# zhuye98/ICL

Hardware: AMD Instinct MI355X
Metric: 3D volumes/sec/node (fwd+bwd, 96^3 patch) (higher is better)
Workload: dtype f32; 1 GPU; 3D U-Net ICL BraTS-shape synthetic 96x96x96, num_classes=2, batch=2 per GPU (1 labeled + 1 unlabeled), full ICL step incl. SGD; global_batch=2, parallelism=dp1, launch=hipGraph replay

## Files before the change

### icl_amd/csrc/icl_abi.inc

```

#include "kernels/common.h"
#include "kernels/norm.h"
#include "kernels/pool_resize.h"
#include "kernels/reduce.h"
#include "kernels/conv_mfma.h"
#include "kernels/conv_mfma_static.h"
#include "kernels/conv_mfma_flat.h"
#include "kernels/conv_bf16x3.h"
#include "kernels/conv_bf16x3_ws.h"
#include "kernels/conv_wgrad_tr.h"
#include "kernels/conv_wgrad_zs.h"
#include "kernels/conv_cin1.h"
#include "kernels/misc.h"
#include "kernels/loss.h"
#include "kernels/optim.h"
#include "kernels/adamw.h"
#include "kernels/winattn.h"
#include "kernels/linear_wgrad.h"
#include "kernels/token.h"
#include "kernels/gemm.h"
#include "kernels/datafeed.h"
#include "kernels/rankindex.h"
#include "kernels/prefix.h"
#include "kernels/intensity.h"
// ... 1760 lines not shown
  ICL_LAUNCH((icl::layernorm_bwd_wgrad_kernel<CPL, RU>), grid, dim3(256), 0, st, gy, x, gamma, mean, rstd, gx, part_g, part_b, (long)rows, c, rpb)
    if (c <= 64) ICL_LN_BW(1, 4);
    else if (c <= 128) ICL_LN_BW(2, 4);
    else if (c <= 256) ICL_LN_BW(4, 2);
    else if (c <= 512) ICL_LN_BW(8, 1);
    else ICL_LN_BW(16, 1);
#undef ICL_LN_BW
    int rc = check_launch("layernorm_bwd_wgrad");
    if (rc || !dgamma) return rc;
    const void* g[2] = {part_g, part_b};
    void* out[2] = {dgamma, dbeta};
    const int32_t rr[2] = {chunks, chunks}, cc[2] = {c, c};
    return icl_colsum_multi(g, out, rr, cc, 2, stream);
  }
  constexpr int longrow = 1;
  if (c >= 1024 && c <= 256 * 64 && longrow) {
    if (c <= 256 * 16) ICL_LAUNCH((icl::layernorm_bwd_longrow_kernel<16>), dim3((unsigned)rows), dim3(256), 0, st, gy, x, gamma, mean, rstd, gx, c);
    else if (c <= 256 * 32) ICL_LAUNCH((icl::layernorm_bwd_longrow_kernel<32>), dim3((unsigned)rows), dim3(256), 0, st, gy, x, gamma, mean, rstd, gx, c);
    else ICL_LAUNCH((icl::layernorm_bwd_longrow_kernel<64>), dim3((unsigned)rows), dim3(256), 0, st, gy, x, gamma, mean, rstd, gx, c);
  } else if (c >= 1024) {
    ICL_LAUNCH((icl::layernorm_bwd_kernel<true>), dim3((unsigned)rows), dim3(256), 0, st, gy, x, gamma, mean, rstd, gx, (long)rows, c);
  } else {
    ICL_LAUNCH((icl::layernorm_bwd_kernel<false>), dim3((unsigned)cdivl(rows, 4)), dim3(256), 0, st, gy, x, gamma, mean, rstd, gx,
               (long)rows, c);
  }
  int rc = check_launch("layernorm_bwd");
  if (rc || !ws) return rc;
  int cols = 256;
  while (cols > c && cols > 16) cols >>= 1;
  if (cols < c && cols < 256) cols <<= 1;
  ICL_LAUNCH(icl::layernorm_wgrad_kernel, dim3((c + cols - 1) / cols, (unsigned)chunks), dim3(256), 0, st, gy, x, mean, rstd, part_g, part_b,
             (long)rows, c, rpb, cols);
  rc = check_launch("layernorm_wgrad");
  if (rc || !dgamma) return rc;
  const void* g[2] = {part_g, part_b};
  void* out[2] = {dgamma, dbeta};
  const int32_t rr[2] = {chunks, chunks}, cc[2] = {c, c};
  return icl_colsum_multi(g, out, rr, cc, 2, stream);
}

int icl_gelu_fwd(const float* x, float* y, int64_t n, void* stream) {
  if (!x || !y || n < 1) return fail(-1, "gelu_fwd: bad argument");
  ICL_LAUNCH(icl::gelu_fwd_kernel, dim3(grid_for(n, 256)), dim3(256), 0, (hipStream_t)stream, x, y, (long)n);
  return check_launch("gelu_fwd");
}

int icl_gelu_bwd(const float* gy, const float* x, float* gx, int64_t n, void* stream) {
  if (!gy || !x || !gx || n < 1) return fail(-1, "gelu_bwd: bad argument");
  ICL_LAUNCH(icl::gelu_bwd_kernel, dim3(grid_for(n, 256)), dim3(256), 0, (hipStream_t)stream, gy, x, gx, (long)n);
  return check_launch("gelu_bwd");
}

static bool attn_class_tiles(int nc) {
  const char* e = getenv("ICL_ATTN_TILED");
  return nc > icl::kAttnMaxNc || (e && atoi(e) == 1);
}

int icl_attn_fwd(const float* q, const float* kv, float* logits, float* out, float* stats, int b, int h, int nc, int n, int d,
                 float scale, void* stream) {
  if (nc < 1 || nc > icl::kAttnMaxClasses) return fail(-1, "attn_fwd: %d classes (1 .. %d)", nc, icl::kAttnMaxClasses);
  if (!q || !kv || !logits || !out || !stats || b < 1 || h < 1 || n < 1 || (d != 8 && d != 16))
    return fail(-1, "attn_fwd: bad argument (head dim 8 or 16)");
  hipStream_t st = (hipStream_t)stream;
  const dim3 g1((n + 255) / 256, b * h), g2(b * h * nc);
  const bool tiled = attn_class_tiles(nc);
  if (d == 16) {
    if (tiled) ICL_LAUNCH((icl::attn_logits_kernel<16, true>), g1, dim3(256), 0, st, q, kv, logits, b, h, nc, n, scale);
    else ICL_LAUNCH((icl::attn_logits_kernel<16, false>), g1, dim3(256), 0, st, q, kv, logits, b, h, nc, n, scale);
    ICL_LAUNCH((icl::attn_softmax_pv_kernel<16, 256>), g2, dim3(256), 0, st, (const float*)logits, kv, out, stats, b, h, nc, n);
  } else {
    if (tiled) ICL_LAUNCH((icl::attn_logits_kernel<8, true>), g1, dim3(256), 0, st, q, kv, logits, b, h, nc, n, scale);
    else ICL_LAUNCH((icl::attn_logits_kernel<8, false>), g1, dim3(256), 0, st, q, kv, logits, b, h, nc, n, scale);
    ICL_LAUNCH((icl::attn_softmax_pv_kernel<8, 256>), g2, dim3(256), 0, st, (const float*)logits, kv, out, stats, b, h, nc, n);
  }
  return check_launch("attn_fwd");
}

int64_t icl_attn_bwd_ws_bytes(int b, int h, int nc, int n, int d) {
  if (b < 1 || h < 1 || nc < 1 || n < 1 || d < 1) return 0;
  return (int64_t)((n + 255) / 256) * b * h * nc * d * 4;
}

int icl_attn_bwd(const float* q, const float* kv, const float* logits, const float* stats, const float* out, const float* gout,
                 const float* glog, float* gq, float* gkv, int b, int h, int nc, int n, int d, float scale, void* stream) {
  return icl_attn_bwd_ws(q, kv, logits, stats, out, gout, glog, gq, gkv, nullptr, b, h, nc, n, d, scale, stream);
}

int icl_attn_bwd_ws(const float* q, const float* kv, const float* logits, const float* stats, const float* out, const float* gout,
                    const float* glog, float* gq, float* gkv, void* ws, int b, int h, int nc, int n, int d, float scale, void* stream) {
  if (nc < 1 || nc > icl::kAttnMaxClasses) return fail(-1, "attn_bwd: %d classes (1 .. %d)", nc, icl::kAttnMaxClasses);
  if (!q || !kv || !logits || !stats || !out || !gq || !gkv || b < 1 || h < 1 || n < 1 || (d != 8 && d != 16))
    return fail(-1, "attn_bwd: bad argument");
  hipStream_t st = (hipStream_t)stream;
  const dim3 g1((n + 255) / 256, b * h), g2(b * h * nc);
  float* pq = (float*)ws;
  const bool tiled = attn_class_tiles(nc);
  if (d == 16) {
    if (tiled) ICL_LAUNCH((icl::attn_bwd_kv_kernel<16, true>), g1, dim3(256), 0, st, q, kv, logits, stats, out, gout, glog, gkv, b, h, nc, n, scale, pq);
    else ICL_LAUNCH((icl::attn_bwd_kv_kernel<16, false>), g1, dim3(256), 0, st, q, kv, logits, stats, out, gout, glog, gkv, b, h, nc, n, scale, pq);
    if (!pq) ICL_LAUNCH((icl::attn_bwd_q_kernel<16, 256>), g2, dim3(256), 0, st, kv, logits, stats, out, gout, glog, gq, b, h, nc, n, scale);
  } else {
    if (tiled) ICL_LAUNCH((icl::attn_bwd_kv_kernel<8, true>), g1, dim3(256), 0, st, q, kv, logits, stats, out, gout, glog, gkv, b, h, nc, n, scale, pq);
    else ICL_LAUNCH((icl::attn_bwd_kv_kernel<8, false>), g1, dim3(256), 0, st, q, kv, logits, stats, out, gout, glog, gkv, b, h, nc, n, scale, pq);
    if (!pq) ICL_LAUNCH((icl::attn_bwd_q_kernel<8, 256>), g2, dim3(256), 0, st, kv, logits, stats, out, gout, glog, gq, b, h, nc, n, scale);
  }
  if (pq) {
    const int rd = b * h * nc * d;
    ICL_LAUNCH(icl::attn_dq_reduce_kernel, dim3((rd + 255) / 256), dim3(256), 0, st, (const float*)pq, gq, (int)g1.x, rd, scale);
  }
  return check_launch("attn_bwd");
}

int64_t icl_window_attn_bias_elems(int n, int heads) { return icl_window_attn_bias_elems_impl(n, heads); }

static int linear_wgrad_nsplit(int64_t rows, int o, int i) {
  const int ob = (o + icl::kLwB - 1) / icl::kLwB, ib = (i + icl::kLwB - 1) / icl::kLwB;
  long n = rows * (o + i) / ((long)o * i + o);
  const long want = (2048 + ob * ib - 1) / (ob * ib);
  if (n > want) n = want;
  const long steps = (rows + 3) / 4;
  if (n > steps / 8) n = steps / 8;
  if (n < 4) n = 4;
  return (int)((n + 3) / 4 * 4);
}

int64_t icl_linear_wgrad_ws_bytes(int64_t rows, int o, int i) {
  return (int64_t)linear_wgrad_nsplit(rows, o, i) * ((int64_t)o * i + o) * 4;
}

int icl_linear_wgrad(const float* gy, const float* x, float* dw, float* db, void* ws, int64_t rows, int o, int i, void* stream) {
  if (!gy || !x || !dw || !ws || rows < 1 || o < 1 || i < 1) return fail(-1, "linear_wgrad: bad argument");
  hipStream_t st = (hipStream_t)stream;
  const int nsplit = linear_wgrad_nsplit(rows, o, i);
  const int ob = (o + icl::kLwB - 1) / icl::kLwB, ib = (i + icl::kLwB - 1) / icl::kLwB;
  ICL_LAUNCH(icl::linear_wgrad_kernel, dim3(nsplit / 4, ob, ib), dim3(256), 0, st, gy, x, (float*)ws, (long)rows, o, i, nsplit);
  if (int rc = check_launch("linear_wgrad")) return rc;
  const long EW = (long)o * i, E = EW + o;
  ICL_LAUNCH(icl::linear_wgrad_reduce_kernel, dim3((unsigned)cdivl(E, 16)), dim3(256), 0, st, (const float*)ws, dw, db, E, EW, nsplit);
  return check_launch("linear_wgrad_reduce");
}

static bool cin1_geom(icl::Cin1Geom& g, int n, int cout, int d, int h, int w, int64_t xbs, int64_t ybs) {
  if (n < 1 || cout < 1 || cout > 16 || d < 1 || h < 1 || w < 1 || (long)d * h * w * 16 >= (1L << 31)) return false;
  g.N = n; g.Cout = cout; g.D = d; g.H = h; g.W = w; g.nty = (h + icl::kC1Rows - 1) / icl::kC1Rows;
  g.x_bstride = xbs; g.y_bstride = ybs; g.ntiles = n * d * g.nty;
  return (size_t)3 * (icl::kC1Rows + 2) * (w + 2) * 4 <= 64 * 1024;
}
static int cin1_grid(const icl::Cin1Geom& g) { return g.ntiles < 2048 ? g.ntiles : 2048; }
static size_t cin1_lds(const icl::Cin1Geom& g) {
  const size_t halo = (size_t)3 * (icl::kC1Rows + 2) * (g.W + 2) * 4;
  return halo > 2048 * 4 ? halo : 2048 * 4;
}

int icl_conv3d_cin1_fwd(const float* x, const float* w, const float* bias, float* y, int n, int cout, int d, int h, int wd, int64_t x_bstride,
                        int64_t y_bstride, void* stream) {
  icl::Cin1Geom g;
  if (!x || !w || !y || !cin1_geom(g, n, cout, d, h, wd, x_bstride, y_bstride)) return fail(-1, "conv3d_cin1_fwd: bad argument");
  ICL_LAUNCH(icl::conv_cin1_fwd_kernel, dim3(cin1_grid(g)), dim3(icl::kC1Threads), cin1_lds(g), (hipStream_t)stream, x, w, bias, y, g);
  snprintf(g_kernel, sizeof(g_kernel), "conv_cin1_fwd_kernel");
  return check_launch("conv3d_cin1_fwd");
}

int64_t icl_conv3d_cin1_wgrad_ws_bytes(int n, int d, int h) {
  const long tiles = (long)n * d * ((h + icl::kC1Rows - 1) / icl::kC1Rows);
  return (tiles < 2048 ? tiles : 2048) * 512 * 4;
}

int icl_conv3d_cin1_wgrad(const float* x, const float* gy, float* gw, void* ws, int n, int cout, int d, int h, int wd, int64_t x_bstride,
                          int64_t gy_bstride, void* stream) {
  icl::Cin1Geom g;
  if (!x || !gy || !gw || !ws || (wd & 3) || (gy_bstride & 3) || !aligned16(gy) || !cin1_geom(g, n, cout, d, h, wd, x_bstride, gy_bstride))
    return fail(-1, "conv3d_cin1_wgrad: bad argument (W and the sample stride of dY must be multiples of 4, dY 16-byte aligned)");
  const int grid = cin1_grid(g);
  ICL_LAUNCH(icl::conv_cin1_wgrad_kernel, dim3(grid), dim3(icl::kC1Threads), cin1_lds(g), (hipStream_t)stream, x, gy, (float*)ws, g);
  if (int rc = check_launch("conv3d_cin1_wgrad")) return rc;
  ICL_LAUNCH(icl::conv_cin1_wgrad_reduce_kernel, dim3(16), dim3(256), 0, (hipStream_t)stream, (const float*)ws, gw, grid, cout);
  snprintf(g_kernel, sizeof(g_kernel), "conv_cin1_wgrad_kernel");
  return check_launch("conv3d_cin1_wgrad_reduce");
}

int64_t icl_conv1x1_wgrad_ws_bytes(int n, int64_t s, int cin, int cout) { return icl_linear_wgrad_ws_bytes((int64_t)n * s, cout, cin); }

namespace {
int conv1x1_wgrad_run(const float* x, const float* gy, float* gw, float* gbias, void* ws, int n, int cin, int cout, int64_t s,
                      int64_t x_bstride, int64_t gy_bstride, const icl::DropSpec& dr, hipStream_t st) {
  const int nsplit = linear_wgrad_nsplit((int64_t)n * s, cout, cin);
  const int ob = (cout + icl::kLwB - 1) / icl::kLwB, ib = (cin + icl::kLwB - 1) / icl::kLwB;
  ICL_LAUNCH(icl::conv1x1_wgrad_kernel, dim3(nsplit / 4, ob, ib), dim3(256), 0, st, gy, x, (float*)ws, n, (long)s, cout, cin, nsplit,
             (long)gy_bstride, (long)x_bstride, dr);
  if (int rc = check_launch("conv1x1_wgrad")) return rc;
  const long EW = (long)cout * cin, E = EW + cout;
  ICL_LAUNCH(icl::linear_wgrad_reduce_kernel, dim3((unsigned)cdivl(E, 16)), dim3(256), 0, st, (const float*)ws, gw, gbias, E, EW, nsplit);
  return check_launch("conv1x1_wgrad_reduce");
}
}

int icl_conv1x1_wgrad(const float* x, const float* gy, float* gw, float* gbias, void* ws, int n, int cin, int cout, int64_t s,
                      int64_t x_bstride, int64_t gy_bstride, void* stream) {
  if (!x || !gy || !gw || !ws || n < 1 || cin < 1 || cout < 1 || s < 4 || (s & 3) || (x_bstride & 3) || (gy_bstride & 3))
    return fail(-1, "conv1x1_wgrad: bad argument (voxel count and batch strides must be multiples of 4)");
  return conv1x1_wgrad_run(x, gy, gw, gbias, ws, n, cin, cout, s, x_bstride, gy_bstride, icl::DropSpec{}, (hipStream_t)stream);
}

int icl_conv1x1_wgrad_dropout(const float* x, const float* gy, float* gw, float* gbias, void* ws, int n, int cin, int cout, int64_t s,
                              int64_t gy_bstride, uint32_t seed, float p, const uint32_t* seed_dev, void* stream) {
  if (!x || !gy || !gw || !ws || n < 1 || cin < 1 || cout < 1 || s < 4 || (s & 3) || (gy_bstride & 3) || !(p >= 0.f && p < 1.f))
    return fail(-1, "conv1x1_wgrad_dropout: bad argument");
  return conv1x1_wgrad_run(x, gy, gw, gbias, ws, n, cin, cout, s, (int64_t)cin * s, gy_bstride, drop_spec(1, seed, p, seed_dev), (hipStream_t)stream);
}

int icl_conv1x1_wgrad_dropout_norm(const float* x, const float* ss, const float* gy, float* gw, float* gbias, void* ws, int n, int cin, int cout,
                                   int64_t s, int64_t gy_bstride, uint32_t seed, float p, const uint32_t* seed_dev, void* stream) {
  if (!x || !ss || !gy || !gw || !ws || n < 1 || cin < 1 || cout < 1 || s < 4 || (s & 3) || (gy_bstride & 3) || !(p >= 0.f && p < 1.f))
    return fail(-1, "conv1x1_wgrad_dropout_norm: bad argument");
  icl::DropSpec dr = p > 0.f ? drop_spec(1, seed, p, seed_dev) : icl::DropSpec{};
  dr.ss = ss;
  return conv1x1_wgrad_run(x, gy, gw, gbias, ws, n, cin, cout, s, (int64_t)cin * s, gy_bstride, dr, (hipStream_t)stream);
}

int icl_relpos_bias_fwd(const float* table, const int64_t* index, float* bias, int n, int heads, int idx_stride, void* stream) {
  if (!table || !index || !bias || n < 1 || n > idx_stride || heads < 1) return fail(-1, "relpos_bias_fwd: bad argument");
  const int npad = (n + 15) / 16 * 16;
  ICL_LAUNCH(icl::relpos_bias_gather_kernel, dim3(grid_for((long)heads * n * npad, 256)), dim3(256), 0, (hipStream_t)stream, table,
             (const long*)index, bias, n, npad, heads, idx_stride);
  return check_launch("relpos_bias_fwd");
}

int icl_window_attn_fwd(const float* qkv, const float* bias, const int32_t* regions, float* out, float* lse, int b_, int n, int heads,
                        int nw, int head_dim, float scale, void* stream) {
  if (!qkv || !bias || !out || !lse) return fail(-1, "window_attn_fwd: null pointer");
  icl::WinAttnGeom g;
  if (int rc = winattn_geom(g, b_, n, heads, nw, head_dim, scale, "window_attn_fwd")) return rc;
  return winattn_fwd_dispatch(qkv, bias, regions, out, lse, g, head_dim, (hipStream_t)stream);
}

int icl_window_attn_bwd(const float* qkv, const float* bias, const int32_t* regions, const float* out, const float* lse,
                        const float* dout, float* dqkv, float* dbias, int b_, int n, int heads, int nw, int head_dim, float scale,
                        void* stream) {
  if (!qkv || !bias || !out || !lse || !dout || !dqkv) return fail(-1, "window_attn_bwd: null pointer");
  icl::WinAttnGeom g;
  if (int rc = winattn_geom(g, b_, n, heads, nw, head_dim, scale, "window_attn_bwd")) return rc;
  return winattn_bwd_dispatch(qkv, bias, regions, out, lse, dout, dqkv, dbias, g, head_dim, (hipStream_t)stream);
}

int icl_window_attn_fwd_drop(const float* qkv, const float* bias, const int32_t* regions, float* out, float* lse, int b_, int n, int heads,
                             int nw, int head_dim, float scale, uint32_t seed, float p, const uint32_t* seed_dev, void* stream) {
  if (!qkv || !bias || !out || !lse) return fail(-1, "window_attn_fwd_drop: null pointer");
  icl::WinAttnGeom g;
  icl::WaDrop d;
  if (int rc = winattn_geom(g, b_, n, heads, nw, head_dim, scale, "window_attn_fwd_drop")) return rc;
  if (int rc = winattn_drop_spec(d, seed, p, seed_dev, "window_attn_fwd_drop")) return rc;
  return winattn_fwd_dispatch(qkv, bias, regions, out, lse, g, head_dim, (hipStream_t)stream, d);
}

int icl_window_attn_bwd_drop(const float* qkv, const float* bias, const int32_t* regions, const float* out, const float* lse,
                             const float* dout, float* dqkv, float* dbias, int b_, int n, int heads, int nw, int head_dim, float scale,
                             uint32_t seed, float p, const uint32_t* seed_dev, void* stream) {
  if (!qkv || !bias || !out || !lse || !dout || !dqkv) return fail(-1, "window_attn_bwd_drop: null pointer");
  icl::WinAttnGeom g;
  icl::WaDrop d;
  if (int rc = winattn_geom(g, b_, n, heads, nw, head_dim, scale, "window_attn_bwd_drop")) return rc;
  if (int rc = winattn_drop_spec(d, seed, p, seed_dev, "window_attn_bwd_drop")) return rc;
  return winattn_bwd_dispatch(qkv, bias, regions, out, lse, dout, dqkv, dbias, g, head_dim, (hipStream_t)stream, d);
}

int icl_window_attn_keep_probe(int32_t* out, int64_t base, int count, uint32_t seed, float p, const uint32_t* seed_dev, void* stream) {
  if (!out || count < 1 || base < 0) return fail(-1, "window_attn_keep_probe: bad argument");
  icl::WaDrop d;
  if (int rc = winattn_drop_spec(d, seed, p, seed_dev, "window_attn_keep_probe")) return rc;
  ICL_LAUNCH(icl::window_attn_keep_probe_kernel, dim3(grid_for(count, 256)), dim3(256), 0, (hipStream_t)stream, (int*)out, (long)base, count, d);
  return check_launch("window_attn_keep_probe");
}

int icl_window_attn_bwd_chunks(int b_, int n, int heads, int nw, int head_dim) {
  icl::WinAttnGeom g;
  if (winattn_geom(g, b_, n, heads, nw, head_dim, 1.f, "window_attn_bwd_chunks")) return 0;
  return winattn_bias_chunks(g);
}

int icl_relpos_bias_bwd_sum(float* dbias, int chunks, const int32_t* inv, const int32_t* offs, float* dtable, int64_t table_rows, int n,
                            int heads, void* stream) {
  if (!dbias || !inv || !offs || !dtable || chunks < 1 || n < 1 || heads < 1 || table_rows < 1)
    return fail(-1, "relpos_bias_bwd_sum: bad argument");
  const int npad = (n + 15) / 16 * 16;
  if (chunks > 1) {
    const long slab = (long)heads * n * npad;
    ICL_LAUNCH(icl::relpos_bias_slab_sum_kernel, dim3(grid_for(slab / 4, 256, 1024)), dim3(256), 0, (hipStream_t)stream, dbias,
               slab, chunks);
    if (int rc = check_launch("relpos_bias_slab_sum")) return rc;
  }
  ICL_LAUNCH(icl::relpos_bias_gather_sum_kernel, dim3((unsigned)((table_rows + 3) / 4), heads), dim3(256), 0, (hipStream_t)stream, dbias, inv,
             offs, dtable, (int)table_rows, n, npad, heads, 1);
  return check_launch("relpos_bias_bwd_sum");
}

int icl_sgd_step(float* p, const float* g, float* m, int64_t n, float lr, float momentum, float weight_decay, int first,
                 const float* lr_dev, void* stream) {
  if (!p || !g || !m || n < 1) return fail(-1, "sgd_step: bad argument");
  ICL_LAUNCH(icl::sgd_momentum_kernel, dim3(grid_for((n + 3) / 4, 256, 4096)), dim3(256), 0, (hipStream_t)stream, p, g, m, (long)n, lr,
             momentum, weight_decay, first, lr_dev);
  return check_launch("sgd_step");
}

int64_t icl_sgd_factored_split_ws_bytes(int rows, int n, int k) {
  if (rows < 1 || n < 1 || k < 1) return 0;
  return (int64_t)3 * ((rows + 7) / 8) * ((int64_t)n + k) * 16;
}

int icl_sgd_step_factored_split(float* p, float* m, const float* g, const float* x, void* ws, int rows, int n, int k, float lr,
                                float momentum, float weight_decay, int first, const float* lr_dev, void* stream) {
  if (!p || !m || !g || !x || !ws || rows < 1 || n < 1 || k < 4 || (k & 3) || !aligned16(ws))
    return fail(-1, "sgd_step_factored_split: bad argument (k %% 4 == 0, workspace of icl_sgd_factored_split_ws_bytes)");
  hipStream_t st = (hipStream_t)stream;
  const int mb = (rows + 7) / 8;
  uint4* gs = (uint4*)ws;
  uint4* xs = gs + (size_t)3 * mb * n;
  ICL_LAUNCH(icl::factor_split_kernel, dim3(grid_for((long)mb * ((long)n + k), 256, 2048)), dim3(256), 0, st, g, x, gs, xs, rows, n, k);
  int rc = check_launch("factor_split");
  if (rc) return rc;
  const size_t lds = (size_t)icl::kSfLdsFloats * 4;
  ICL_SET_MAX_DYN_LDS(icl::sgd_factored_split_kernel, kMaxDynLdsBig);
  ICL_LAUNCH(icl::sgd_factored_split_kernel, dim3((k + icl::kSfCols - 1) / icl::kSfCols, (n + icl::kSfRows - 1) / icl::kSfRows), dim3(256), lds,
             st, p, m, (const uint4*)gs, (const uint4*)xs, rows, n, k, lr, momentum, weight_decay, first, lr_dev);
  return check_launch("sgd_step_factored_split");
}

// ... 1570 lines not shown
```

### icl_amd/csrc/kernels/conv_cin1.h

```cpp
#pragma once

namespace icl {

constexpr int kC1Rows = 8, kC1Threads = 256;

struct Cin1Geom {
  int N, Cout, D, H, W, nty;
  long x_bstride, y_bstride;
  int ntiles;
};

__device__ __forceinline__ void c1_stage_halo(float* xs, const float* __restrict__ x, const Cin1Geom& g, int n, int z, int y0) {
  const int PW = g.W + 2, PR = kC1Rows + 2;
  const long HW = (long)g.H * g.W;
  const float* xb = x + (long)n * g.x_bstride;
  for (int it = threadIdx.x; it < 3 * PR * PW; it += kC1Threads) {
    const int px = it % PW, row = it / PW, py = row % PR, pz = row / PR;
    const int gz = z - 1 + pz, gy = y0 - 1 + py, gx = px - 1;
    float v = 0.f;
    if ((unsigned)gz < (unsigned)g.D && (unsigned)gy < (unsigned)g.H && (unsigned)gx < (unsigned)g.W) v = xb[gz * HW + (long)gy * g.W + gx];
    xs[it] = v;
  }
}

__global__ __launch_bounds__(kC1Threads) void conv_cin1_wgrad_kernel(const float* __restrict__ x, const float* __restrict__ gy,
                                                                     float* __restrict__ part, Cin1Geom g) {
  ICL_DYN_LDS(float, xs);
  const int lane = threadIdx.x & 63, wid = threadIdx.x >> 6, lr = lane & 15, lg = lane >> 4;
  const int PW = g.W + 2, PR = kC1Rows + 2;
  const long HW = (long)g.H * g.W, DHW = g.D * HW;
  int toff[2];
  bool tok[2];
#pragma unroll
  for (int tb = 0; tb < 2; ++tb) {
    const int tap = 16 * tb + lr;
    tok[tb] = tap < 27;
    const int t = tok[tb] ? tap : 0;
    toff[tb] = (t / 9) * PR * PW + ((t / 3) % 3) * PW + t % 3;
  }
  f32x4 acc[2] = {f32x4{0.f, 0.f, 0.f, 0.f}, f32x4{0.f, 0.f, 0.f, 0.f}};
  for (int tile = blockIdx.x; tile < g.ntiles; tile += gridDim.x) {
    const int n = tile / (g.D * g.nty), rem = tile % (g.D * g.nty), z = rem / g.nty, y0 = (rem % g.nty) * kC1Rows;
    __syncthreads();
    c1_stage_halo(xs, x, g, n, z, y0);
    __syncthreads();
    const float* gb = gy + (long)n * g.y_bstride + (long)lr * DHW + (long)z * HW;
    for (int rr = 0; rr < 2; ++rr) {
      const int ty = 2 * wid + rr, yy = y0 + ty;
      if (yy >= g.H) break;
      const float* grow = gb + (long)yy * g.W;
      const float* xrow = xs + (ty * PW);
      for (int x0 = 0; x0 < g.W; x0 += 16) {
        const int xl = x0 + 4 * lg;
        float4 a = make_float4(0.f, 0.f, 0.f, 0.f);
        if (lr < g.Cout && xl < g.W) a = *reinterpret_cast<const float4*>(grow + xl);
        const float av[4] = {a.x, a.y, a.z, a.w};
        const bool in = xl < g.W;
#pragma unroll
        for (int j = 0; j < 4; ++j) {
#pragma unroll
          for (int tb = 0; tb < 2; ++tb) {
            const float b = (tok[tb] && in) ? xrow[toff[tb] + xl + j] : 0.f;
            acc[tb] = icl_mfma_16x16x4(av[j], b, acc[tb]);
          }
        }
      }
    }
  }
  __syncthreads();
  float* red = xs;
#pragma unroll
  for (int tb = 0; tb < 2; ++tb)
#pragma unroll
    for (int r = 0; r < 4; ++r) red[((wid * 2 + tb) * 4 + r) * 64 + lane] = acc[tb][r];
  __syncthreads();
  if (wid == 0) {
#pragma unroll
    for (int tb = 0; tb < 2; ++tb)
#pragma unroll
      for (int r = 0; r < 4; ++r) {
        float s = 0.f;
#pragma unroll
        for (int w = 0; w < 4; ++w) s += red[((w * 2 + tb) * 4 + r) * 64 + lane];
        part[(long)blockIdx.x * 512 + (4 * lg + r) * 32 + 16 * tb + lr] = s;
      }
  }
}

__global__ __launch_bounds__(256) void conv_cin1_wgrad_reduce_kernel(const float* __restrict__ part, float* __restrict__ gw, int nparts, int cout) {
  __shared__ float sl[8][32];
  const int o = threadIdx.x & 31, slice = threadIdx.x >> 5, e = blockIdx.x * 32 + o;
  float s = 0.f;
#pragma unroll 8
  for (int p = slice; p < nparts; p += 8) s += part[(long)p * 512 + e];
  sl[slice][o] = s;
  __syncthreads();
  if (slice == 0) {
    float t = 0.f;
#pragma unroll
    for (int k = 0; k < 8; ++k) t += sl[k][o];
    const int co = e >> 5, tap = e & 31;
    if (co < cout && tap < 27) gw[co * 27 + tap] = t;
  }
}

__global__ __launch_bounds__(kC1Threads) void conv_cin1_fwd_kernel(const float* __restrict__ x, const float* __restrict__ w,
                                                                   const float* __restrict__ bias, float* __restrict__ y, Cin1Geom g) {
  ICL_DYN_LDS(float, xs);
  const int lane = threadIdx.x & 63, wid = threadIdx.x >> 6, lr = lane & 15, lg = lane >> 4;
  const int PW = g.W + 2, PR = kC1Rows + 2;
  const long HW = (long)g.H * g.W, DHW = g.D * HW;
  float wa[7];
  int toff[7];
#pragma unroll
  for (int s = 0; s < 7; ++s) {
    const int tap = 4 * s + lg;
    wa[s] = (tap < 27 && lr < g.Cout) ? w[lr * 27 + tap] : 0.f;
    const int t = tap < 27 ? tap : 0;
    toff[s] = (t / 9) * PR * PW + ((t / 3) % 3) * PW + t % 3;
  }
  float bv[4];
#pragma unroll
  for (int r = 0; r < 4; ++r) bv[r] = (bias && 4 * lg + r < g.Cout) ? bias[4 * lg + r] : 0.f;
  for (int tile = blockIdx.x; tile < g.ntiles; tile += gridDim.x) {
    const int n = tile / (g.D * g.nty), rem = tile % (g.D * g.nty), z = rem / g.nty, y0 = (rem % g.nty) * kC1Rows;
    __syncthreads();
    c1_stage_halo(xs, x, g, n, z, y0);
    __syncthreads();
    float* yb = y + (long)n * g.y_bstride + (long)z * HW;
    for (int rr = 0; rr < 2; ++rr) {
      const int ty = 2 * wid + rr, yy = y0 + ty;
      if (yy >= g.H) break;
      const float* xrow = xs + ty * PW;
      for (int x0 = 0; x0 < g.W; x0 += 16) {
        const int xp = x0 + lr;
        const bool in = xp < g.W;
        f32x4 acc = f32x4{bv[0], bv[1], bv[2], bv[3]};
#pragma unroll
        for (int s = 0; s < 7; ++s) acc = icl_mfma_16x16x4(wa[s], in ? xrow[toff[s] + xp] : 0.f, acc);
        if (in) {
#pragma unroll
          for (int r = 0; r < 4; ++r)
            if (4 * lg + r < g.Cout) yb[(long)(4 * lg + r) * DHW + (long)yy * g.W + xp] = acc[r];
        }
      }
    }
  }
}

}
```

Measured before the change: 210.6 volumes/s.

## Stream z-planes through an LDS ring buffer in Cin=1 conv fwd and wgrad

Adds streaming variants of the single-input-channel 3D conv forward and weight-gradient kernels. Each block walks consecutive z-slices of a fixed y-tile and keeps a 4-slot ring of halo planes in LDS, so each new tile loads only one new plane (prefetched into registers during compute) instead of restaging all three. It also vectorises the halo and output stores and double-buffers dY loads in wgrad. The cost is more complex tile scheduling and more LDS per block, and the host still sizes the wgrad reduce by the old grid.

```diff
diff --git a/icl_amd/csrc/icl_abi.inc b/icl_amd/csrc/icl_abi.inc
--- a/icl_amd/csrc/icl_abi.inc
+++ b/icl_amd/csrc/icl_abi.inc
@@ -1936,10 +1936,30 @@
   return halo > 2048 * 4 ? halo : 2048 * 4;
 }
 
+static size_t cin1_ring_bytes(const icl::Cin1Geom& g) { return (size_t)4 * (icl::kC1Rows + 2) * (((g.W + 3) & ~3) + 8) * 4; }
+static bool cin1_stream(const icl::Cin1Geom& g) { return env_int("ICL_CONV_CIN1_STREAM", 1) != 0 && cin1_ring_bytes(g) <= 64 * 1024; }
+static bool cin1_x_vec(const icl::Cin1Geom& g, const float* x) { return !(g.W & 3) && !(g.x_bstride & 3) && aligned16(x); }
+static icl::Cin1Walk cin1_plan(const icl::Cin1Geom& g, int P, int tmax, int lmax, int cap) {
+  icl::Cin1Walk k = icl::cin1_walk(g, P, 1, lmax);
+  for (int t = 2; t <= tmax && k.nb * g.nty > cap; ++t) k = icl::cin1_walk(g, P, t, lmax);
+  return k;
+}
+
 int icl_conv3d_cin1_fwd(const float* x, const float* w, const float* bias, float* y, int n, int cout, int d, int h, int wd, int64_t x_bstride,
                         int64_t y_bstride, void* stream) {
   icl::Cin1Geom g;
   if (!x || !w || !y || !cin1_geom(g, n, cout, d, h, wd, x_bstride, y_bstride)) return fail(-1, "conv3d_cin1_fwd: bad argument");
+  if (cin1_stream(g)) {
+    const icl::Cin1Walk wk = cin1_plan(g, g.ntiles, 8, 8, 1024);
+    const dim3 grid(wk.nb * g.nty), block(icl::kC1Threads);
+    const int vec = cin1_x_vec(g, x);
+    if (!(g.W & 3) && !(g.y_bstride & 3) && aligned16(y))
+      ICL_LAUNCH(icl::conv_cin1_fwd_stream_kernel<true>, grid, block, cin1_ring_bytes(g), (hipStream_t)stream, x, w, bias, y, g, wk, vec);
+    else
+      ICL_LAUNCH(icl::conv_cin1_fwd_stream_kernel<false>, grid, block, cin1_ring_bytes(g), (hipStream_t)stream, x, w, bias, y, g, wk, vec);
+    snprintf(g_kernel, sizeof(g_kernel), "conv_cin1_fwd_kernel");
+    return check_launch("conv3d_cin1_fwd");
+  }
   ICL_LAUNCH(icl::conv_cin1_fwd_kernel, dim3(cin1_grid(g)), dim3(icl::kC1Threads), cin1_lds(g), (hipStream_t)stream, x, w, bias, y, g);
   snprintf(g_kernel, sizeof(g_kernel), "conv_cin1_fwd_kernel");
   return check_launch("conv3d_cin1_fwd");
@@ -1956,6 +1976,16 @@
   if (!x || !gy || !gw || !ws || (wd & 3) || (gy_bstride & 3) || !aligned16(gy) || !cin1_geom(g, n, cout, d, h, wd, x_bstride, gy_bstride))
     return fail(-1, "conv3d_cin1_wgrad: bad argument (W and the sample stride of dY must be multiples of 4, dY 16-byte aligned)");
   const int grid = cin1_grid(g);
+  if (cin1_stream(g)) {
+    const icl::Cin1Walk wk = icl::cin1_walk(g, grid, 1, 1);
+    const size_t ring = cin1_ring_bytes(g);
+    ICL_LAUNCH((icl::conv_cin1_wgrad_stream_kernel<1, 6>), dim3(wk.nb * g.nty), dim3(icl::kC1Threads), ring > 8192 ? ring : 8192,
+               (hipStream_t)stream, x, gy, (float*)ws, g, wk, (int)cin1_x_vec(g, x));
+    if (int rc = check_launch("conv3d_cin1_wgrad")) return rc;
+    ICL_LAUNCH(icl::conv_cin1_wgrad_reduce_kernel, dim3(16), dim3(256), 0, (hipStream_t)stream, (const float*)ws, gw, grid, cout);
+    snprintf(g_kernel, sizeof(g_kernel), "conv_cin1_wgrad_kernel");
+    return check_launch("conv3d_cin1_wgrad_reduce");
+  }
   ICL_LAUNCH(icl::conv_cin1_wgrad_kernel, dim3(grid), dim3(icl::kC1Threads), cin1_lds(g), (hipStream_t)stream, x, gy, (float*)ws, g);
   if (int rc = check_launch("conv3d_cin1_wgrad")) return rc;
   ICL_LAUNCH(icl::conv_cin1_wgrad_reduce_kernel, dim3(16), dim3(256), 0, (hipStream_t)stream, (const float*)ws, gw, grid, cout);
diff --git a/icl_amd/csrc/kernels/conv_cin1.h b/icl_amd/csrc/kernels/conv_cin1.h
--- a/icl_amd/csrc/kernels/conv_cin1.h
+++ b/icl_amd/csrc/kernels/conv_cin1.h
@@ -148,4 +148,368 @@
   }
 }
 
-}
+
+constexpr int kC1MaxChains = 4;
+constexpr int kC1PfQuads = 2;
+
+struct Cin1Walk {
+  int P, rounds, cmax, cA, LA, LB, nbA, nb;
+};
+
+static inline Cin1Walk cin1_walk(const Cin1Geom& g, int P, int T, int lmax) {
+  Cin1Walk k;
+  k.P = P;
+  k.rounds = (g.ntiles + P - 1) / P;
+  k.cmax = (P + g.nty - 1) / g.nty;
+  const int R = g.ntiles - (k.rounds - 1) * P;
+  k.cA = R >= P ? k.cmax : (R + g.nty - 1) / g.nty;
+  auto clampl = [lmax](int v) { return v < 1 ? 1 : (v > lmax ? lmax : v); };
+  k.LA = clampl(T / k.rounds);
+  k.LB = clampl(k.rounds > 1 ? T / (k.rounds - 1) : T);
+  k.nbA = (k.cA + k.LA - 1) / k.LA;
+  k.nb = k.nbA + (k.cmax - k.cA + k.LB - 1) / k.LB;
+  return k;
+}
+
+struct C1Ring {
+  int PWs, PS;
+  __device__ __forceinline__ explicit C1Ring(int W) : PWs(((W + 3) & ~3) + 8), PS((kC1Rows + 2) * PWs) {}
+};
+
+struct C1Cursor {
+  int k, i, t, n, z, y0;
+  bool valid;
+};
+
+struct C1Seq {
+  int yt, c0, nch, P, rounds, ntiles, nty, D;
+  __device__ __forceinline__ C1Seq(const Cin1Geom& g, const Cin1Walk& w, int b) {
+    const int blk = b / g.nty;
+    yt = b - blk * g.nty;
+    int L;
+    if (blk < w.nbA) {
+      c0 = blk * w.LA;
+      L = w.cA - c0 < w.LA ? w.cA - c0 : w.LA;
+    } else {
+      c0 = w.cA + (blk - w.nbA) * w.LB;
+      L = w.LB;
+    }
+    nch = 0;
+    for (int i = 0; i < L; ++i) nch += ((c0 + i) * g.nty + yt < w.P) ? 1 : 0;
+    P = w.P; rounds = w.rounds; ntiles = g.ntiles; nty = g.nty; D = g.D;
+  }
+  __device__ __forceinline__ int chain(int i) const { return (c0 + i) * nty + yt; }
+  __device__ __forceinline__ C1Cursor round(int k) const {
+    C1Cursor c;
+    c.k = k; c.i = 0;
+    const long t = (long)chain(0) + (long)k * P;
+    c.valid = k < rounds && nch > 0 && t < ntiles;
+    c.t = c.valid ? (int)t : 0;
+    const int nz = c.t / nty;
+    c.y0 = (c.t - nz * nty) * kC1Rows;
+    c.n = nz / D;
+    c.z = nz - c.n * D;
+    return c;
+  }
+  __device__ __forceinline__ C1Cursor first() const { return round(0); }
+  __device__ __forceinline__ C1Cursor next(C1Cursor c) const {
+    if (c.i + 1 < nch && c.t + nty < ntiles) {
+      ++c.i;
+      c.t += nty;
+      if (++c.z == D) {
+        c.z = 0;
+        ++c.n;
+      }
+      return c;
+    }
+    return round(c.k + 1);
+  }
+};
+
+struct C1Items {
+  int py[kC1PfQuads], go[kC1PfQuads], lo[kC1PfQuads];
+  __device__ __forceinline__ C1Items(const Cin1Geom& g, const C1Ring& rg) {
+    const int nq = g.W >> 2, items = nq ? (kC1Rows + 2) * nq : 0;
+#pragma unroll
+    for (int u = 0; u < kC1PfQuads; ++u) {
+      const int it = threadIdx.x + u * kC1Threads, p = nq ? it / nq : 0, q = it - p * nq;
+      py[u] = p;
+      go[u] = (p - 1) * g.W + 4 * q;
+      lo[u] = it < items ? p * rg.PWs + 4 + 4 * q : -1;
+    }
+  }
+};
+__device__ __forceinline__ void c1s_plane_load(float4 (&r)[kC1PfQuads], const C1Items& im, const float* __restrict__ xb, const Cin1Geom& g,
+                                               int zp, int y0) {
+  const float* base = xb + ((long)zp * g.H + y0) * g.W;
+  const bool zin = (unsigned)zp < (unsigned)g.D;
+#pragma unroll
+  for (int u = 0; u < kC1PfQuads; ++u) {
+    r[u] = make_float4(0.f, 0.f, 0.f, 0.f);
+    if (zin && im.lo[u] >= 0 && (unsigned)(y0 - 1 + im.py[u]) < (unsigned)g.H) r[u] = *reinterpret_cast<const float4*>(base + im.go[u]);
+  }
+}
+__device__ __forceinline__ void c1s_plane_store(float* xs, const C1Ring& rg, const float4 (&r)[kC1PfQuads], const C1Items& im, int zp) {
+  float* slot = xs + (zp & 3) * rg.PS;
+#pragma unroll
+  for (int u = 0; u < kC1PfQuads; ++u)
+    if (im.lo[u] >= 0) *reinterpret_cast<float4*>(slot + im.lo[u]) = r[u];
+}
+__device__ __forceinline__ void c1s_plane_rest(float* xs, const C1Ring& rg, const float* __restrict__ xb, const Cin1Geom& g, int zp, int y0,
+                                               bool vec) {
+  float* slot = xs + (zp & 3) * rg.PS;
+  const bool zin = (unsigned)zp < (unsigned)g.D;
+  if (vec) {
+    const int nq = g.W >> 2, items = (kC1Rows + 2) * nq;
+    for (int it = kC1PfQuads * kC1Threads + threadIdx.x; it < items; it += kC1Threads) {
+      const int py = it / nq, q = it - py * nq, gy = y0 - 1 + py;
+      float4 v = make_float4(0.f, 0.f, 0.f, 0.f);
+      if (zin && (unsigned)gy < (unsigned)g.H) v = *reinterpret_cast<const float4*>(xb + ((long)zp * g.H + gy) * g.W + 4 * q);
+      *reinterpret_cast<float4*>(slot + py * rg.PWs + 4 + 4 * q) = v;
+    }
+  } else {
+    const int items = (kC1Rows + 2) * g.W;
+    for (int it = threadIdx.x; it < items; it += kC1Threads) {
+      const int py = it / g.W, gx = it - py * g.W, gy = y0 - 1 + py;
+      float v = 0.f;
+      if (zin && (unsigned)gy < (unsigned)g.H) v = xb[((long)zp * g.H + gy) * g.W + gx];
+      slot[py * rg.PWs + 4 + gx] = v;
+    }
+  }
+}
+__device__ __forceinline__ void c1s_stage3(float* xs, const C1Ring& rg, const C1Items& im, const float* __restrict__ xb, const Cin1Geom& g,
+                                           int z, int y0, bool vec) {
+  if (vec) {
+    float4 r[3][kC1PfQuads];
+#pragma unroll
+    for (int d = 0; d < 3; ++d) c1s_plane_load(r[d], im, xb, g, z - 1 + d, y0);
+#pragma unroll
+    for (int d = 0; d < 3; ++d) c1s_plane_store(xs, rg, r[d], im, z - 1 + d);
+  }
+  if (!vec || (kC1Rows + 2) * (g.W >> 2) > kC1PfQuads * kC1Threads)
+    for (int d = 0; d < 3; ++d) c1s_plane_rest(xs, rg, xb, g, z - 1 + d, y0, vec);
+}
+
+template <class TileFn>
+__device__ __forceinline__ void c1s_walk(float* xs, const C1Ring& rg, const float* __restrict__ x, const Cin1Geom& g, const C1Seq& sq,
+                                         bool vec, TileFn&& tile) {
+  for (int it = threadIdx.x; it < 4 * rg.PS; it += kC1Threads) xs[it] = 0.f;
+  C1Cursor cur = sq.first();
+  if (!cur.valid) return;
+  const C1Items im(g, rg);
+  const bool rest = !vec || (kC1Rows + 2) * (g.W >> 2) > kC1PfQuads * kC1Threads;
+  __syncthreads();
+  c1s_stage3(xs, rg, im, x + (long)cur.n * g.x_bstride, g, cur.z, cur.y0, vec);
+  __syncthreads();
+  for (;;) {
+    const C1Cursor nx = sq.next(cur);
+    const bool pf = nx.valid && nx.n == cur.n && nx.y0 == cur.y0 && nx.z == cur.z + 1;
+    const float* xb = x + (long)cur.n * g.x_bstride;
+    float4 pr[kC1PfQuads];
+    if (pf && vec) c1s_plane_load(pr, im, xb, g, cur.z + 2, cur.y0);
+    tile(cur);
+    if (pf) {
+      if (vec) c1s_plane_store(xs, rg, pr, im, cur.z + 2);
+      if (rest) c1s_plane_rest(xs, rg, xb, g, cur.z + 2, cur.y0, vec);
+    }
+    __syncthreads();
+    if (!nx.valid) break;
+    if (!pf) {
+      c1s_stage3(xs, rg, im, x + (long)nx.n * g.x_bstride, g, nx.z, nx.y0, vec);
+      __syncthreads();
+    }
+    cur = nx;
+  }
+}
+
+template <bool kT>
+__global__ __launch_bounds__(kC1Threads) void conv_cin1_fwd_stream_kernel(const float* __restrict__ x, const float* __restrict__ w,
+                                                                          const float* __restrict__ bias, float* __restrict__ y, Cin1Geom g,
+                                                                          Cin1Walk wk, int vec) {
+  ICL_DYN_LDS(float, xs);
+  const int lane = threadIdx.x & 63, lr = lane & 15, lg = lane >> 4;
+  int wid = threadIdx.x >> 6;
+  ICL_WAVE_UNIFORM(wid);
+  const C1Ring rg(g.W);
+  const long HW = (long)g.H * g.W, DHW = g.D * HW;
+  float wa[7];
+  int tdz[7], toff[7];
+#pragma unroll
+  for (int s = 0; s < 7; ++s) {
+    const int tap = 4 * s + lg;
+    wa[s] = (tap < 27 && lr < g.Cout) ? w[lr * 27 + tap] : 0.f;
+    const int t = tap < 27 ? tap : 0;
+    tdz[s] = t / 9;
+    toff[s] = ((t / 3) % 3) * rg.PWs + t % 3 + 3;
+  }
+  float bv[4];
+#pragma unroll
+  for (int r = 0; r < 4; ++r) {
+    const int co = kT ? lr : 4 * lg + r;
+    bv[r] = (bias && co < g.Cout) ? bias[co] : 0.f;
+  }
+  const C1Seq sq(g, wk, blockIdx.x);
+  c1s_walk(xs, rg, x, g, sq, vec != 0, [&](const C1Cursor& c) {
+    float* yb = y + (long)c.n * g.y_bstride + (long)c.z * HW;
+    int off[7];
+#pragma unroll
+    for (int s = 0; s < 7; ++s) off[s] = ((c.z - 1 + tdz[s]) & 3) * rg.PS + toff[s];
+    for (int rr = 0; rr < 2; ++rr) {
+      const int ty = 2 * wid + rr, yy = c.y0 + ty;
+      if (yy >= g.H) break;
+      const float* xrow = xs + ty * rg.PWs;
+      for (int x0 = 0; x0 < g.W; x0 += 16) {
+        const int xp = x0 + lr;
+        const bool in = xp < g.W;
+        f32x4 acc = f32x4{bv[0], bv[1], bv[2], bv[3]};
+        if (kT) {
+#pragma unroll
+          for (int s = 0; s < 7; ++s) acc = icl_mfma_16x16x4(in ? xrow[off[s] + xp] : 0.f, wa[s], acc);
+          const int xl = x0 + 4 * lg;
+          if (xl < g.W && lr < g.Cout)
+            *reinterpret_cast<float4*>(yb + (long)lr * DHW + (long)yy * g.W + xl) = make_float4(acc[0], acc[1], acc[2], acc[3]);
+        } else {
+#pragma unroll
+          for (int s = 0; s < 7; ++s) acc = icl_mfma_16x16x4(wa[s], in ? xrow[off[s] + xp] : 0.f, acc);
+          if (in) {
+#pragma unroll
+            for (int r = 0; r < 4; ++r)
+              if (4 * lg + r < g.Cout) yb[(long)(4 * lg + r) * DHW + (long)yy * g.W + xp] = acc[r];
+          }
+        }
+      }
+    }
+  });
+}
+
+template <int B>
+struct C1Batch {
+  float4 v[B];
+};
+struct C1WaveCursor {
+  C1Cursor t;
+  int rr, xb;
+};
+__device__ __forceinline__ void c1s_wave_settle(C1WaveCursor& p, const C1Seq& sq, const Cin1Geom& g, int wid) {
+  while (p.t.valid && (p.rr >= 2 || p.t.y0 + 2 * wid + p.rr >= g.H)) {
+    p.t = sq.next(p.t);
+    p.rr = 0;
+    p.xb = 0;
+  }
+}
+__device__ __forceinline__ void c1s_wave_advance(C1WaveCursor& p, const C1Seq& sq, const Cin1Geom& g, int wid, int step) {
+  p.xb += step;
+  if (p.xb >= g.W) {
+    p.xb = 0;
+    ++p.rr;
+  }
+  c1s_wave_settle(p, sq, g, wid);
+}
+template <int B>
+__device__ __forceinline__ void c1s_batch_load(C1Batch<B>& b, const C1WaveCursor& p, const float* __restrict__ gy, const Cin1Geom& g, int wid,
+                                               int lr, int lg) {
+  const long HW = (long)g.H * g.W, DHW = g.D * HW;
+  const float* grow = gy + (long)p.t.n * g.y_bstride + (long)lr * DHW + (long)p.t.z * HW + (long)(p.t.y0 + 2 * wid + p.rr) * g.W;
+#pragma unroll
+  for (int u = 0; u < B; ++u) {
+    const int xl = p.xb + 16 * u + 4 * lg;
+    b.v[u] = make_float4(0.f, 0.f, 0.f, 0.f);
+    if (p.t.valid && lr < g.Cout && xl < g.W) b.v[u] = *reinterpret_cast<const float4*>(grow + xl);
+  }
+}
+
+template <int NC, int B>
+__global__ __launch_bounds__(kC1Threads) void conv_cin1_wgrad_stream_kernel(const float* __restrict__ x, const float* __restrict__ gy,
+                                                                            float* __restrict__ part, Cin1Geom g, Cin1Walk wk, int vec) {
+  ICL_DYN_LDS(float, xs);
+  const int lane = threadIdx.x & 63, lr = lane & 15, lg = lane >> 4;
+  int wid = threadIdx.x >> 6;
+  ICL_WAVE_UNIFORM(wid);
+  const C1Ring rg(g.W);
+  int tdz[2], toff[2];
+  bool tok[2];
+#pragma unroll
+  for (int tb = 0; tb < 2; ++tb) {
+    const int tap = 16 * tb + lr;
+    tok[tb] = tap < 27;
+    const int t = tok[tb] ? tap : 0;
+    tdz[tb] = t / 9;
+    toff[tb] = ((t / 3) % 3) * rg.PWs + t % 3 + 3;
+  }
+  const f32x4 zero4 = f32x4{0.f, 0.f, 0.f, 0.f};
+  f32x4 accs[NC][2];
+#pragma unroll
+  for (int u = 0; u < NC; ++u) accs[u][0] = accs[u][1] = zero4;
+  const C1Seq sq(g, wk, blockIdx.x);
+  C1WaveCursor pc;
+  pc.t = sq.first();
+  pc.rr = 0;
+  pc.xb = 0;
+  c1s_wave_settle(pc, sq, g, wid);
+  C1Batch<B> cb;
+  c1s_batch_load(cb, pc, gy, g, wid, lr, lg);
+  c1s_wave_advance(pc, sq, g, wid, 16 * B);
+  c1s_walk(xs, rg, x, g, sq, vec != 0, [&](const C1Cursor& c) {
+    f32x4 a0 = zero4, a1 = zero4;
+#pragma unroll
+    for (int u = 0; u < NC; ++u)
+      if (u == c.i) { a0 = accs[u][0]; a1 = accs[u][1]; }
+    int off[2];
+#pragma unroll
+    for (int tb = 0; tb < 2; ++tb) off[tb] = ((c.z - 1 + tdz[tb]) & 3) * rg.PS + toff[tb];
+    for (int rr = 0; rr < 2; ++rr) {
+      const int ty = 2 * wid + rr, yy = c.y0 + ty;
+      if (yy >= g.H) break;
+      const float* xrow = xs + ty * rg.PWs;
+      for (int xb = 0; xb < g.W; xb += 16 * B) {
+        C1Batch<B> nb;
+        c1s_batch_load(nb, pc, gy, g, wid, lr, lg);
+        c1s_wave_advance(pc, sq, g, wid, 16 * B);
+#pragma unroll
+        for (int u = 0; u < B; ++u) {
+          const int x0 = xb + 16 * u;
+          if (x0 < g.W) {
+            const int xl = x0 + 4 * lg;
+            const float av[4] = {cb.v[u].x, cb.v[u].y, cb.v[u].z, cb.v[u].w};
+            const bool in = xl < g.W;
+#pragma unroll
+            for (int j = 0; j < 4; ++j) {
+              a0 = icl_mfma_16x16x4(av[j], (tok[0] && in) ? xrow[off[0] + xl + j] : 0.f, a0);
+              a1 = icl_mfma_16x16x4(av[j], (tok[1] && in) ? xrow[off[1] + xl + j] : 0.f, a1);
+            }
+          }
+        }
+        cb = nb;
+      }
+    }
+#pragma unroll
+    for (int u = 0; u < NC; ++u)
+      if (u == c.i) { accs[u][0] = a0; accs[u][1] = a1; }
+  });
+  __syncthreads();
+  float* red = xs;
+#pragma unroll
+  for (int u = 0; u < NC; ++u)
+    if (u < sq.nch) {
+#pragma unroll
+      for (int tb = 0; tb < 2; ++tb)
+#pragma unroll
+        for (int r = 0; r < 4; ++r) red[u * 2048 + ((wid * 2 + tb) * 4 + r) * 64 + lane] = accs[u][tb][r];
+    }
+  __syncthreads();
+  if (wid < sq.nch) {
+    const float* rc = red + wid * 2048;
+    float* pp = part + (long)sq.chain(wid) * 512;
+#pragma unroll
+    for (int tb = 0; tb < 2; ++tb)
+#pragma unroll
+      for (int r = 0; r < 4; ++r) {
+        float s = 0.f;
+#pragma unroll
+        for (int w = 0; w < 4; ++w) s += rc[((w * 2 + tb) * 4 + r) * 64 + lane];
+        pp[(4 * lg + r) * 32 + 16 * tb + lr] = s;
+      }
+  }
+}
+
+}
```

Result: no change. 210.5 volumes/s (-0.1%).
